# YuHang-max/3DSAD-main

Hardware: AMD Instinct MI355X
Metric: scenes/sec (16384-pt KITTI-shaped) through SA+cluster path (higher is better)
Workload: dtype f32

## Files before the change

### 3dsad-main_amd/csrc/ball_query.hip

```cpp
#include "common.h"

namespace {

struct BQParams {
    float radii[SAD_MAX_RADII];
    int nsample[SAD_MAX_RADII];
    int32_t *idx[SAD_MAX_RADII];
    int32_t *cnt[SAD_MAX_RADII];
};

constexpr int BQ_WAVES = 4;

template <int NR, int CW>
__global__ __launch_bounds__(BQ_WAVES * 64) void ball_query_kernel(
    const float *__restrict__ xyz, const float *__restrict__ new_xyz,
    const float *__restrict__ radius_pc, BQParams prm, int N, int M) {
    const int lane = threadIdx.x & 63;
    const int wave = __builtin_amdgcn_readfirstlane(threadIdx.x >> 6);
    const int b = blockIdx.y;
    const int m0 = (blockIdx.x * BQ_WAVES + wave) * CW;
    const float *p = xyz + (size_t)b * N * 3;

    float cx[CW], cy[CW], cz[CW], r2[CW][NR];
    int cnt[CW][NR], first[CW][NR];
    bool active[CW];
    int ndone = 0;
#pragma unroll
    for (int c = 0; c < CW; ++c) {
        active[c] = (m0 + c) < M;
        const int m = active[c] ? m0 + c : M - 1;
        const float *q = new_xyz + ((size_t)b * M + m) * 3;
        cx[c] = q[0];
        cy[c] = q[1];
        cz[c] = q[2];
#pragma unroll
        for (int r = 0; r < NR; ++r) {
            float rad = prm.radii[r];
            if (radius_pc) rad = rad * radius_pc[(size_t)b * M + m];
            r2[c][r] = rad * rad;
            first[c][r] = 0;
            cnt[c][r] = active[c] ? 0 : prm.nsample[r];
            if (!active[c]) ++ndone;
        }
    }

    for (int base = 0; base < N && ndone < CW * NR; base += 64) {
        const int j = base + lane;
        const bool valid = j < N;
        const int jj = valid ? j : N - 1;
        const float px = p[jj * 3 + 0], py = p[jj * 3 + 1], pz = p[jj * 3 + 2];
#pragma unroll
        for (int c = 0; c < CW; ++c) {
            const float d = sad::d2f(px, py, pz, cx[c], cy[c], cz[c]);
#pragma unroll
            for (int r = 0; r < NR; ++r) {
                const bool in = valid && (d < r2[c][r]);
                const unsigned long long mask = __ballot(in);
                if (mask != 0ull && cnt[c][r] < prm.nsample[r]) {
                    const int slot = cnt[c][r] + __builtin_amdgcn_mbcnt_hi((unsigned)(mask >> 32), __builtin_amdgcn_mbcnt_lo((unsigned)mask, 0u));
                    if (in && slot < prm.nsample[r])
                        prm.idx[r][((size_t)b * M + (m0 + c)) * prm.nsample[r] + slot] = j;
                    if (cnt[c][r] == 0) first[c][r] = base + __builtin_ctzll(mask);
                    cnt[c][r] += __builtin_popcountll(mask);
                    if (cnt[c][r] >= prm.nsample[r]) ++ndone;
                }
            }
        }
    }
#pragma unroll
    for (int c = 0; c < CW; ++c) {
        if (!active[c]) continue;
#pragma unroll
        for (int r = 0; r < NR; ++r) {
            const int S = prm.nsample[r];
            const int n = cnt[c][r] < S ? cnt[c][r] : S;
            for (int s = n + lane; s < S; s += 64)
                prm.idx[r][((size_t)b * M + (m0 + c)) * S + s] = first[c][r];
            if (prm.cnt[r] && lane == 0) prm.cnt[r][(size_t)b * M + (m0 + c)] = n;
        }
    }
}

template <int NR>
void launch_bq(const float *xyz, const float *new_xyz, const float *radius_pc, const BQParams &prm,
               int B, int N, int M, hipStream_t st) {
    constexpr int CW = 4;
    dim3 grid((M + BQ_WAVES * CW - 1) / (BQ_WAVES * CW), B);
    hipLaunchKernelGGL((ball_query_kernel<NR, CW>), grid, dim3(BQ_WAVES * 64), 0, st, xyz, new_xyz,
                       radius_pc, prm, N, M);
}

__global__ __launch_bounds__(256) void knn_kernel(const float *__restrict__ xyz,
                                                  const float *__restrict__ new_xyz, int N, int M,
                                                  int K, int32_t *__restrict__ idx) {
    const int lane = threadIdx.x & 63;
    const int wave = __builtin_amdgcn_readfirstlane(threadIdx.x >> 6);
    const int b = blockIdx.y;
    const int m = blockIdx.x * 4 + wave;
    if (m >= M) return;
    const float *p = xyz + (size_t)b * N * 3;
    const float *q = new_xyz + ((size_t)b * M + m) * 3;
    const float cx = q[0], cy = q[1], cz = q[2];
    float ld = __builtin_inff();
    int lj = 0;
    float worst = __builtin_inff();
    int filled = 0;
    for (int base = 0; base < N; base += 64) {
        const int j = base + lane;
        const bool valid = j < N;
        const int jj = valid ? j : N - 1;
        const float d = sad::d2f(p[jj * 3 + 0], p[jj * 3 + 1], p[jj * 3 + 2], cx, cy, cz);
        unsigned long long mask = __ballot(valid && (d < worst || filled < K));
        while (mask) {
            const int l = __builtin_ctzll(mask);
            mask &= mask - 1;
            const float xd = __builtin_bit_cast(float, __builtin_amdgcn_readlane(__builtin_bit_cast(int, d), l));
            if (!(xd < worst) && filled >= K) continue;
            const int pos = __builtin_popcountll(__ballot(lane < filled && ld <= xd));
            const float ud = __shfl_up(ld, 1, 64);
            const int uj = __shfl_up(lj, 1, 64);
            if (lane > pos) {
                ld = ud;
                lj = uj;
            } else if (lane == pos) {
                ld = xd;
                lj = base + l;
            }
            if (lane >= K) ld = __builtin_inff();
            filled = filled < K ? filled + 1 : K;
            worst = filled < K ? __builtin_inff() : __builtin_bit_cast(float, __builtin_amdgcn_readlane(__builtin_bit_cast(int, ld), K - 1));
        }
    }
    if (lane < K) idx[((size_t)b * M + m) * K + lane] = lj;
}

int check_common(const char *fn, const void *xyz, const void *new_xyz, int B, int N, int M) {
    if (!xyz || !new_xyz) return sad::fail(SAD_EINVAL, "%s: NULL pointer", fn);
    if (B < 1 || N < 1 || M < 1) return sad::fail(SAD_EINVAL, "%s: need B,N,M >= 1 (B=%d N=%d M=%d)", fn, B, N, M);
    if (B > 65535) return sad::fail(SAD_EUNSUPPORTED, "%s: B=%d > 65535", fn, B);
    if ((size_t)N * 3 >= (1u << 31)) return sad::fail(SAD_EUNSUPPORTED, "%s: N too large", fn);
    return SAD_OK;
}

}

SAD_API int sad_ball_query_multi_f32(const float *xyz, const float *new_xyz, int n_radii,
                                     const float *radii, const float *radius_pc,
                                     const int *nsamples, int32_t *const *idx, int32_t *const *cnt,
                                     int B, int N, int M, sad_stream_t stream) {
    if (int e = check_common("sad_ball_query_multi_f32", xyz, new_xyz, B, N, M)) return e;
    SAD_REQUIRE(n_radii >= 1 && n_radii <= SAD_MAX_RADII, "sad_ball_query_multi_f32: n_radii=%d not in 1..%d", n_radii, SAD_MAX_RADII);
    SAD_REQUIRE(radii && nsamples && idx, "sad_ball_query_multi_f32: NULL parameter array");
    BQParams prm{};
    for (int r = 0; r < n_radii; ++r) {
        SAD_REQUIRE(nsamples[r] >= 1 && nsamples[r] <= 64, "sad_ball_query: nsample=%d not in 1..64", nsamples[r]);
        SAD_REQUIRE(idx[r], "sad_ball_query: NULL idx output");
        prm.radii[r] = radii[r];
        prm.nsample[r] = nsamples[r];
        prm.idx[r] = idx[r];
        prm.cnt[r] = cnt ? cnt[r] : nullptr;
    }
    hipStream_t st = (hipStream_t)stream;
    switch (n_radii) {
        case 1: launch_bq<1>(xyz, new_xyz, radius_pc, prm, B, N, M, st); break;
        case 2: launch_bq<2>(xyz, new_xyz, radius_pc, prm, B, N, M, st); break;
        case 3: launch_bq<3>(xyz, new_xyz, radius_pc, prm, B, N, M, st); break;
        default: launch_bq<4>(xyz, new_xyz, radius_pc, prm, B, N, M, st); break;
    }
    return sad::check_launch("sad_ball_query");
}

SAD_API int sad_ball_query_f32(const float *xyz, const float *new_xyz, float radius,
                               const float *radius_pc, int B, int N, int M, int S, int32_t *idx,
                               sad_stream_t stream) {
    const float radii[1] = {radius_pc ? 1.0f : radius};
    const int ns[1] = {S};
    int32_t *const outs[1] = {idx};
    return sad_ball_query_multi_f32(xyz, new_xyz, 1, radii, radius_pc, ns, outs, nullptr, B, N, M, stream);
}

SAD_API int sad_knn_f32(const float *xyz, const float *new_xyz, int B, int N, int M, int K,
                        int32_t *idx, sad_stream_t stream) {
    if (int e = check_common("sad_knn_f32", xyz, new_xyz, B, N, M)) return e;
    SAD_REQUIRE(idx, "sad_knn_f32: NULL idx");
    SAD_REQUIRE(K >= 1 && K <= 64 && K <= N, "sad_knn_f32: need 1 <= K <= min(64, N) (K=%d N=%d)", K, N);
    dim3 grid((M + 3) / 4, B);
    hipLaunchKernelGGL(knn_kernel, grid, dim3(256), 0, (hipStream_t)stream, xyz, new_xyz, N, M, K, idx);
    return sad::check_launch("sad_knn_f32");
}
```

Baseline: 8461.

## Stage small point clouds in LDS as SoA and prefetch in ball query

Measured after the change: 8561, median of 6. 1.01x the previous value.

```diff
diff --git a/3dsad-main_amd/csrc/ball_query.hip b/3dsad-main_amd/csrc/ball_query.hip
--- a/3dsad-main_amd/csrc/ball_query.hip
+++ b/3dsad-main_amd/csrc/ball_query.hip
@@ -9,19 +9,53 @@
     int32_t *cnt[SAD_MAX_RADII];
 };
 
-constexpr int BQ_WAVES = 4;
-
-template <int NR, int CW>
+constexpr int BQ_WAVES = 8;
+constexpr int BQ_CW = 2;
+constexpr int BQ_BLOCK = BQ_WAVES * BQ_CW;
+constexpr int BQ_STAGE_MAX = 2048;
+constexpr int BQ_STAGE_LOADS = BQ_STAGE_MAX / (BQ_WAVES * 64);
+
+template <int NR, int CW, bool STAGED>
 __global__ __launch_bounds__(BQ_WAVES * 64) void ball_query_kernel(
     const float *__restrict__ xyz, const float *__restrict__ new_xyz,
     const float *__restrict__ radius_pc, BQParams prm, int N, int M) {
+    extern __shared__ float bq_lds[];
     const int lane = threadIdx.x & 63;
     const int wave = __builtin_amdgcn_readfirstlane(threadIdx.x >> 6);
     const int b = blockIdx.y;
+    const float *p = xyz + (size_t)b * N * 3;
+    const int Np = (N + 63) & ~63;
+    const float *sx = bq_lds, *sy = bq_lds + Np, *sz = bq_lds + 2 * Np;
+
+    if (STAGED) {
+        float vx[BQ_STAGE_LOADS], vy[BQ_STAGE_LOADS], vz[BQ_STAGE_LOADS];
+#pragma unroll
+        for (int k = 0; k < BQ_STAGE_LOADS; ++k) {
+            if (k * BQ_WAVES * 64 >= Np) break;
+            const int j = k * BQ_WAVES * 64 + (int)threadIdx.x;
+            const int jj = j < N ? j : N - 1;
+            vx[k] = p[jj * 3 + 0];
+            vy[k] = p[jj * 3 + 1];
+            vz[k] = p[jj * 3 + 2];
+        }
+#pragma unroll
+        for (int k = 0; k < BQ_STAGE_LOADS; ++k) {
+            if (k * BQ_WAVES * 64 >= Np) break;
+            const int j = k * BQ_WAVES * 64 + (int)threadIdx.x;
+            if (j < Np) {
+                const bool real = j < N;
+                bq_lds[j] = real ? vx[k] : __builtin_nanf("");
+                bq_lds[Np + j] = real ? vy[k] : __builtin_nanf("");
+                bq_lds[2 * Np + j] = real ? vz[k] : __builtin_nanf("");
+            }
+        }
+        __syncthreads();
+    }
+
     const int m0 = (blockIdx.x * BQ_WAVES + wave) * CW;
-    const float *p = xyz + (size_t)b * N * 3;
-
-    float cx[CW], cy[CW], cz[CW], r2[CW][NR];
+    if (m0 >= M) return;
+
+    float cx[CW], cy[CW], cz[CW], r2[CW][NR], rw[CW];
     int cnt[CW][NR], first[CW][NR];
     bool active[CW];
     int ndone = 0;
@@ -33,30 +67,50 @@
         cx[c] = q[0];
         cy[c] = q[1];
         cz[c] = q[2];
+        rw[c] = -__builtin_inff();
 #pragma unroll
         for (int r = 0; r < NR; ++r) {
             float rad = prm.radii[r];
             if (radius_pc) rad = rad * radius_pc[(size_t)b * M + m];
             r2[c][r] = rad * rad;
+            rw[c] = r2[c][r] > rw[c] ? r2[c][r] : rw[c];
             first[c][r] = 0;
             cnt[c][r] = active[c] ? 0 : prm.nsample[r];
             if (!active[c]) ++ndone;
         }
     }
 
+    float px, py, pz;
+    if (STAGED) {
+        px = sx[lane];
+        py = sy[lane];
+        pz = sz[lane];
+    }
     for (int base = 0; base < N && ndone < CW * NR; base += 64) {
         const int j = base + lane;
-        const bool valid = j < N;
-        const int jj = valid ? j : N - 1;
-        const float px = p[jj * 3 + 0], py = p[jj * 3 + 1], pz = p[jj * 3 + 2];
+        const bool valid = STAGED || j < N;
+        float qx, qy, qz;
+        if (STAGED) {
+            const int jn = base + 64 < Np ? j + 64 : j;
+            qx = sx[jn];
+            qy = sy[jn];
+            qz = sz[jn];
+        } else {
+            const int jj = valid ? j : N - 1;
+            px = p[jj * 3 + 0];
+            py = p[jj * 3 + 1];
+            pz = p[jj * 3 + 2];
+        }
 #pragma unroll
         for (int c = 0; c < CW; ++c) {
             const float d = sad::d2f(px, py, pz, cx[c], cy[c], cz[c]);
+            if (__ballot(valid && (d < rw[c])) == 0ull) continue;
 #pragma unroll
             for (int r = 0; r < NR; ++r) {
+                if (cnt[c][r] >= prm.nsample[r]) continue;
                 const bool in = valid && (d < r2[c][r]);
                 const unsigned long long mask = __ballot(in);
-                if (mask != 0ull && cnt[c][r] < prm.nsample[r]) {
+                if (mask != 0ull) {
                     const int slot = cnt[c][r] + __builtin_amdgcn_mbcnt_hi((unsigned)(mask >> 32), __builtin_amdgcn_mbcnt_lo((unsigned)mask, 0u));
                     if (in && slot < prm.nsample[r])
                         prm.idx[r][((size_t)b * M + (m0 + c)) * prm.nsample[r] + slot] = j;
@@ -66,6 +120,11 @@
                 }
             }
         }
+        if (STAGED) {
+            px = qx;
+            py = qy;
+            pz = qz;
+        }
     }
 #pragma unroll
     for (int c = 0; c < CW; ++c) {
@@ -84,10 +143,10 @@
 template <int NR>
 void launch_bq(const float *xyz, const float *new_xyz, const float *radius_pc, const BQParams &prm,
                int B, int N, int M, hipStream_t st) {
-    constexpr int CW = 4;
-    dim3 grid((M + BQ_WAVES * CW - 1) / (BQ_WAVES * CW), B);
-    hipLaunchKernelGGL((ball_query_kernel<NR, CW>), grid, dim3(BQ_WAVES * 64), 0, st, xyz, new_xyz,
-                       radius_pc, prm, N, M);
+    dim3 grid((M + BQ_BLOCK - 1) / BQ_BLOCK, B);
+    const size_t lds = N <= BQ_STAGE_MAX ? (size_t)3 * ((N + 63) & ~63) * sizeof(float) : 0;
+    auto kernel = N <= BQ_STAGE_MAX ? ball_query_kernel<NR, BQ_CW, true> : ball_query_kernel<NR, BQ_CW, false>;
+    hipLaunchKernelGGL(kernel, grid, dim3(BQ_WAVES * 64), lds, st, xyz, new_xyz, radius_pc, prm, N, M);
 }
 
 __global__ __launch_bounds__(256) void knn_kernel(const float *__restrict__ xyz,
```
